# vlc-robot/robot-3dlotus

Hardware: AMD Instinct MI355X
Metric: keystep-samples/sec (train fwd+bwd) 3D-LOTUS GemBench (higher is better)
Workload: dtype f32; 1 GPU; 3D-LOTUS v1 (68.18M params), 16 key-step clouds x 4096 pts per GPU, fwd+loss+bwd, train mode (dropout on), fp32 exact (MFMA f32); global_batch=16, parallelism=dp1, rccl_ranks=0

## Files before the change

robot-3dlotus_amd/csrc/attention.hip:

```cpp
#include "mma.h"
#include <stdlib.h>

namespace LOTUS_NS {

#define AT 128
#define ALD 33
#define SLD 129

struct AttnP {
  const act_t* q; long q_ld; int q_off;
  const act_t* kv; long kv_ld; int k_off, v_off;
  const int* qidx;
  const int* kidx;
  const int* owner;
  const int* tiles;
  const int* blocks;
  const float* qn_w; const float* qn_b; const float* kn_w; const float* kn_b;
  act_t* out; long out_ld;
  float* lse;
  const act_t* dout;
  act_t* dq; long dq_ld; int dq_off;
  act_t* dkv; long dkv_ld; int dk_off, dv_off; long dkv_part_stride;
  float* ln_part;
  int atomic_out;
  const int* kext;
  act_t* dkv_extra;
  long dkv_extra_ld;
  int H, d;
  float scale, eps;
  unsigned long long drop_seed;
  unsigned drop_thresh;
  float drop_inv_keep;
};

__device__ __forceinline__ bool keep_lo(unsigned lo, unsigned s0, unsigned c2, unsigned thresh) {
  unsigned x = lo * 0x9E3779B1u + s0;
  x ^= c2;
  x ^= x >> 16; x *= 0x7FEB352Du; x ^= x >> 15;
  return x >= thresh;
}

__device__ __forceinline__ f32x16 zero16() {
  f32x16 z;
#pragma unroll
  for (int r = 0; r < 16; ++r) z[r] = 0.f;
  return z;
}

// ... 47 lines not shown
  }
  float* x = img + row * ALD;
  float m = 0.f;
  for (int j = 0; j < d; ++j) m += x[j];
  m /= d;
  float v = 0.f;
  for (int j = 0; j < d; ++j) {
    const float c = x[j] - m;
    v += c * c;
  }
  const float rs = rsqrtf(v / d + eps);
  rstd_s[row] = rs;
  for (int j = 0; j < d; ++j) {
    const float xh = (x[j] - m) * rs;
    x[j] = AFFINE ? xh * g_s[j] + b_s[j] : xh;
  }
}

struct AttnSmem {
  float* Q; float* K; float* V; float* dO; float* S;
  float* qrstd; float* krstd; float* Dv; float* lse;
  float* gq; float* bq; float* gk; float* bk;
  int* qrow; int* krow; int* qown; int* kext;
};

__device__ __forceinline__ AttnSmem carve(float* base, bool bwd) {
  AttnSmem s;
  float* p = base;
  s.Q = p; p += AT * ALD;
  s.K = p; p += AT * ALD;
// ... 43 lines not shown
    else
      l[q] = 0u;
  }
  hi = make_uint4(h[0], h[1], h[2], h[3]);
  lo = make_uint4(l[0], l[1], l[2], l[3]);
}
template <int PREC>
__device__ __forceinline__ f32x16 mfma_split(const uint4& ah, const uint4& al, const uint4& bh, const uint4& bl, f32x16 acc) {
  if (PREC == 3) {
    acc = __builtin_amdgcn_mfma_f32_32x32x16_bf16(__builtin_bit_cast(abf16x8, al), __builtin_bit_cast(abf16x8, bh), acc, 0, 0, 0);
    acc = __builtin_amdgcn_mfma_f32_32x32x16_bf16(__builtin_bit_cast(abf16x8, ah), __builtin_bit_cast(abf16x8, bl), acc, 0, 0, 0);
  }
  return __builtin_amdgcn_mfma_f32_32x32x16_bf16(__builtin_bit_cast(abf16x8, ah), __builtin_bit_cast(abf16x8, bh), acc, 0, 0, 0);
}

template <int PREC, bool NORM = true>
__global__ __launch_bounds__(256, 3) void attn_fwd_kernel(AttnP p) {
  static_assert(NORM || PREC == 0, "the no-norm variant exists in exact fp32 only");
  extern __shared__ __attribute__((aligned(16))) float smem[];
  AttnSmem s = carve(smem, false);
  const int tid = threadIdx.x, wave = tid >> 6, l31 = tid & 31, hh = (tid >> 5) & 1;
  const int h = blockIdx.y, d = p.d;
  const int q_start = p.tiles[blockIdx.x * 4 + 0], q_len = p.tiles[blockIdx.x * 4 + 1];
  const int k_start = p.tiles[blockIdx.x * 4 + 2], k_len = p.tiles[blockIdx.x * 4 + 3];

  if (tid < AT) {
    s.qrow[tid] = tid < q_len ? (p.qidx ? p.qidx[q_start + tid] : q_start + tid) : -1;
    s.krow[tid] = tid < k_len ? (p.kidx ? p.kidx[k_start + tid] : k_start + tid) : -1;
    s.qown[tid] = tid < q_len ? (p.owner ? p.owner[q_start + tid] : 1) : 0;
  }
  if constexpr (NORM) load_affine(p, s);
  __syncthreads();
  {
    const RowSrc src[3] = {{s.Q, p.q, p.q_ld, p.q_off + h * d, s.qrow, q_len}, {s.K, p.kv, p.kv_ld, p.k_off + h * d, s.krow, k_len},
                           {s.V, p.kv, p.kv_ld, p.v_off + h * d, s.krow, k_len}};
    load_rows_batch<3>(src, d);
  }
  __syncthreads();
  if constexpr (NORM) {
    if (tid < AT) ln_rows<true>(s.Q, s.qrstd, tid, q_len, d, p.eps, s.gq, s.bq);
    else ln_rows<true>(s.K, s.krstd, tid - AT, k_len, d, p.eps, s.gk, s.bk);
    __syncthreads();
  }

  const int r0 = wave * 32;
  if (r0 >= q_len) return;
  const int ktiles = (k_len + 31) / 32;
  const int qi = r0 + l31;
  f32x16 acc[4];
#pragma unroll
  for (int t = 0; t < 4; ++t) acc[t] = zero16();
  if constexpr (PREC != 0) {
    uint4 qh[2], ql[2];
#pragma unroll
    for (int q2 = 0; q2 < 2; ++q2) {
      float v[8];
#pragma unroll
      for (int e = 0; e < 8; ++e) v[e] = s.Q[qi * ALD + q2 * 16 + hh * 8 + e];
// ... 31 lines not shown
      acc[t][r] = v;
      m = fmaxf(m, v);
    }
  m = fmaxf(m, __shfl_xor(m, 32, 64));
  float sum = 0.f;
#pragma unroll
  for (int t = 0; t < 4; ++t)
#pragma unroll
    for (int r = 0; r < 16; ++r) {
      const float e = acc[t][r] > -INFINITY ? __expf(acc[t][r] - m) : 0.f;
      acc[t][r] = e;
      sum += e;
    }
  sum += __shfl_xor(sum, 32, 64);
  const float inv = sum > 0.f ? 1.f / sum : 0.f;
  if (p.drop_thresh) {
    const unsigned long long rb = (((unsigned long long)blockIdx.x * p.H + h) * AT + qi) * AT;
    const unsigned lo0 = (unsigned)rb, c2 = (unsigned)(rb >> 32) * 0x7FEB352Du + (unsigned)(p.drop_seed >> 32);
    const unsigned s0 = (unsigned)p.drop_seed;
    const float keep = inv * p.drop_inv_keep;
#pragma unroll
    for (int t = 0; t < 4; ++t)
#pragma unroll
      for (int r = 0; r < 16; ++r)
        acc[t][r] *= keep_lo(lo0 + (unsigned)(t * 32 + (r & 3) + 8 * (r >> 2) + 4 * hh), s0, c2, p.drop_thresh) ? keep : 0.f;
  } else {
#pragma unroll
    for (int t = 0; t < 4; ++t)
#pragma unroll
      for (int r = 0; r < 16; ++r) acc[t][r] *= inv;
// ... 21 lines not shown
#pragma unroll
        for (int r = 0; r < 16; ++r) {
          const int key = t * 32 + (r & 3) + 8 * (r >> 2) + 4 * hh;
          o = __builtin_amdgcn_mfma_f32_32x32x2f32(s.V[key * ALD + l31], acc[t][r], o, 0, 0, 0);
        }
      }
    }
  if (qi < q_len && s.qown[qi]) {
    act_t* orow = p.out + (long)s.qrow[qi] * p.out_ld + h * d;
#pragma unroll
    for (int q4 = 0; q4 < 4; ++q4) {
      const int dc = 8 * q4 + 4 * hh;
      if (dc < d) st4(orow + dc, make_float4(o[4 * q4], o[4 * q4 + 1], o[4 * q4 + 2], o[4 * q4 + 3]));
    }
  }
}

__device__ __forceinline__ void store_rows(const float* img, act_t* base, long ld, int coff, const int* rows_s,
                                           const int* own_s, int len, int d, int atomic, const int* ext_s = nullptr,
                                           act_t* ext_base = nullptr, long ext_ld = 0, int ext_coff = 0) {
  const int sub = threadIdx.x & 7;
  for (int r = threadIdx.x >> 3; r < len; r += 32) {
    if (own_s && !own_s[r]) continue;
    if (sub * 4 >= d) continue;
    const float* v = img + r * ALD + sub * 4;
    act_t* o = base + (long)rows_s[r] * ld + coff + sub * 4;
    if (ext_s && ext_s[r] >= 0) o = ext_base + (long)ext_s[r] * ext_ld + ext_coff + sub * 4;
#if !LOTUS_ACT_IS_BF16
    if (atomic) {
#pragma unroll
// ... 8 lines not shown
__device__ __forceinline__ void ln_rows_bwd(float* g, const float* xh, const float* rstd_s, int row, int len, int d,
                                            const float* gam) {
  if (row >= len) return;
  float* gr = g + row * ALD;
  const float* xr = xh + row * ALD;
  float s1 = 0.f, s2 = 0.f;
  for (int j = 0; j < d; ++j) {
    const float t = gr[j] * gam[j];
    s1 += t;
    s2 += t * xr[j];
  }
  s1 /= d;
  s2 /= d;
  const float rs = rstd_s[row];
  for (int j = 0; j < d; ++j) gr[j] = rs * (gr[j] * gam[j] - s1 - xr[j] * s2);
}

template <int PREC>
__global__ __launch_bounds__(256, 2) void attn_bwd_kernel(AttnP p) {
  extern __shared__ __attribute__((aligned(16))) float smem[];
  AttnSmem s = carve(smem, true);
  __shared__ float lnacc[4][32];
  __shared__ float colred[2][8][32];
  const int tid = threadIdx.x, wave = tid >> 6, l31 = tid & 31, hh = (tid >> 5) & 1;
  const int h = blockIdx.y, d = p.d;
  const int* bd = p.blocks + blockIdx.x * 6;
  const int first_tile = bd[0], n_tiles = bd[1], tile_step = bd[2], part_slot = bd[3];
  const int k_start = bd[4], k_len = bd[5];
  const int r0 = wave * 32;
  const int ktiles = (k_len + 31) / 32;
// ... 352 lines not shown
  }
  if (tid < AT) ln_rows_bwd(s.dO, s.K, s.krstd, tid, k_len, d, s.gk);
  __syncthreads();
  act_t* dkv = p.dkv + (long)part_slot * p.dkv_part_stride;
  store_rows(s.dO, dkv, p.dkv_ld, p.dk_off + h * d, s.krow, nullptr, k_len, d, p.atomic_out, p.dkv_extra ? s.kext : nullptr,
             p.dkv_extra, p.dkv_extra_ld, h * d);
  store_rows(s.V, dkv, p.dkv_ld, p.dv_off + h * d, s.krow, nullptr, k_len, d, p.atomic_out, p.dkv_extra ? s.kext : nullptr,
             p.dkv_extra, p.dkv_extra_ld, p.dv_off - p.dk_off + h * d);
  if (tid < 128) p.ln_part[((long)(blockIdx.x * p.H + h) * 4 + (tid >> 5)) * 32 + (tid & 31)] = lnacc[tid >> 5][tid & 31];
}

typedef float f32x4v __attribute__((ext_vector_type(4)));

__device__ __forceinline__ int xswz(int key) { return ((key & 1) << 2) | ((key >> 1) & 3); }

template <bool NORM = true>
__global__ __launch_bounds__(256, 2) void attn_bwd2_kernel(AttnP p) {
  extern __shared__ __attribute__((aligned(16))) float smem[];
  AttnSmem s = carve(smem, true);
  __shared__ float lnacc[NORM ? 4 : 1][32];
  __shared__ float colred[NORM ? 2 : 1][NORM ? 8 : 1][32];
  const int tid = threadIdx.x, wave = tid >> 6, lane = tid & 63, l31 = tid & 31, hh = (tid >> 5) & 1;
  const int h = blockIdx.y, d = p.d;
  const int* bd = p.blocks + blockIdx.x * 6;
  const int first_tile = bd[0], n_tiles = bd[1], tile_step = bd[2], part_slot = bd[3];
  const int k_start = bd[4], k_len = bd[5];
  const int r0 = wave * 32;
  const int ktiles = (k_len + 31) / 32;
  float* X = s.V;

  if (tid < AT) {
    s.krow[tid] = tid < k_len ? (p.kidx ? p.kidx[k_start + tid] : k_start + tid) : -1;
    s.kext[tid] = (tid < k_len && p.kext) ? p.kext[k_start + tid] : -1;
  }
  if constexpr (NORM) {
    if (tid < 4 * 32) lnacc[tid >> 5][tid & 31] = 0.f;
    load_affine(p, s);
  }
  __syncthreads();
  {
    const RowSrc src[2] = {{s.K, p.kv, p.kv_ld, p.k_off + h * d, s.krow, k_len}, {s.V, p.kv, p.kv_ld, p.v_off + h * d, s.krow, k_len}};
    load_rows_batch<2>(src, d);
  }
  __syncthreads();
  if constexpr (NORM) {
    if (tid >= AT) ln_rows<false>(s.K, s.krstd, tid - AT, k_len, d, p.eps, nullptr, nullptr);
    __syncthreads();
  }

  const float gq_l = NORM ? s.gq[l31] : 1.f, bq_l = NORM ? s.bq[l31] : 0.f;
  const float sl2 = p.scale * 1.4426950408889634f;
  const bool has_keys = r0 < k_len;
  const int kj = r0 + l31;
  float kb[16], vb[16], c_a = 0.f;
  if (has_keys) {
#pragma unroll
    for (int s2 = 0; s2 < 16; ++s2) {
      const int k = 2 * s2 + hh;
      if constexpr (NORM) {
        const float kn = s.K[kj * ALD + k] * s.gk[k] + s.bk[k];
        c_a += s.bq[k] * kn;
        kb[s2] = kn * s.gq[k] * sl2;
      } else {
        kb[s2] = s.K[kj * ALD + k] * sl2;
      }
      vb[s2] = s.V[kj * ALD + k];
    }
    if constexpr (NORM) {
      c_a += __shfl_xor(c_a, 32, 64);
      c_a = kj < k_len ? c_a * sl2 : -INFINITY;
    } else {
      c_a = kj < k_len ? 0.f : -INFINITY;
    }
  }
  f32x16 acc_dv = zero16(), acc_dk = zero16();
  const int dh = wave & 1, qh = wave >> 1, l15 = lane & 15, kq = lane >> 4;
  const float gk_c = NORM ? s.gk[16 * dh + l15] : 1.f, bk_c = NORM ? s.bk[16 * dh + l15] : 0.f;
  __syncthreads();

  for (int ti = 0; ti < n_tiles; ++ti) {
    const int tile = first_tile + ti * tile_step;
    const int q_start = p.tiles[tile * 4 + 0], q_len = p.tiles[tile * 4 + 1];
    if (tid < AT) {
      s.qrow[tid] = tid < q_len ? (p.qidx ? p.qidx[q_start + tid] : q_start + tid) : -1;
      s.qown[tid] = tid < q_len ? (p.owner ? p.owner[q_start + tid] : 1) : 0;
      s.lse[tid] = tid < q_len ? p.lse[(long)(q_start + tid) * p.H + h] * 1.4426950408889634f : INFINITY;
    }
    __syncthreads();
    {
      const int sub = tid & 7, rr0 = tid >> 3;
      float4 qv[4], gv[4], ov[4];
#pragma unroll
      for (int j = 0; j < 4; ++j) {
        const int r = rr0 + 32 * j;
        qv[j] = gv[j] = ov[j] = make_float4(0.f, 0.f, 0.f, 0.f);
        if (r < q_len && sub * 4 < d) {
          qv[j] = ld4(p.q + (long)s.qrow[r] * p.q_ld + p.q_off + h * d + sub * 4);
          if (s.qown[r]) {
            const long o = (long)s.qrow[r] * p.out_ld + h * d + sub * 4;
            gv[j] = ld4(p.dout + o);
            ov[j] = ld4(p.out + o);
          }
        }
      }
#pragma unroll
      for (int j = 0; j < 4; ++j) {
        const int r = rr0 + 32 * j;
        float* oq = s.Q + r * ALD + sub * 4;
        oq[0] = qv[j].x; oq[1] = qv[j].y; oq[2] = qv[j].z; oq[3] = qv[j].w;
        float* o = s.dO + r * ALD + sub * 4;
        o[0] = gv[j].x; o[1] = gv[j].y; o[2] = gv[j].z; o[3] = gv[j].w;
        float dsum = gv[j].x * ov[j].x + gv[j].y * ov[j].y + gv[j].z * ov[j].z + gv[j].w * ov[j].w;
        dsum += __shfl_xor(dsum, 1, 64);
        dsum += __shfl_xor(dsum, 2, 64);
        dsum += __shfl_xor(dsum, 4, 64);
        if (sub == 0) s.Dv[r] = dsum;
      }
    }
    __syncthreads();
    if constexpr (NORM) {
      if (tid < AT) ln_rows<false>(s.Q, s.qrstd, tid, q_len, d, p.eps, nullptr, nullptr);
      __syncthreads();
    }

    const unsigned long long tb = ((unsigned long long)tile * p.H + h) * AT * AT;
    const unsigned c2 = (unsigned)(tb >> 32) * 0x7FEB352Du + (unsigned)(p.drop_seed >> 32);
    const unsigned x_lane = ((unsigned)tb + (unsigned)kj + (unsigned)(4 * hh * AT)) * 0x9E3779B1u + (unsigned)p.drop_seed;
    const int qtiles = (q_len + 31) / 32;
    for (int qt = 0; qt < qtiles; ++qt) {
      f32x16 sa, dpa;
      if (has_keys) {
#pragma unroll
        for (int r = 0; r < 16; ++r) { sa[r] = c_a; dpa[r] = 0.f; }
        const float* qrow_p = s.Q + (qt * 32 + l31) * ALD + hh;
        const float* dorow_p = s.dO + (qt * 32 + l31) * ALD + hh;
#pragma unroll
        for (int s2 = 0; s2 < 16; ++s2) {
          sa = __builtin_amdgcn_mfma_f32_32x32x2f32(qrow_p[2 * s2], kb[s2], sa, 0, 0, 0);
// ... 50 lines not shown
        const float* kcol = s.K + 16 * dh + l15;
        for (int t = 0; t < ktiles; ++t) {
#pragma unroll
          for (int s4 = 0; s4 < 8; ++s4) {
            const int key = 32 * t + 4 * s4 + kq;
            const float a = NORM ? kcol[key * ALD] * gk_c + bk_c : kcol[key * ALD];
            const float b = X[key * 32 + ((((ql >> 2) ^ xswz(key)) << 2) | (ql & 3))];
            acc = __builtin_amdgcn_mfma_f32_16x16x4f32(a, b, acc, 0, 0, 0);
          }
        }
        float* o = s.dO + (qt * 32 + ql) * ALD + 16 * dh + 4 * kq;
        o[0] = acc[0]; o[1] = acc[1]; o[2] = acc[2]; o[3] = acc[3];
      }
    }
    __syncthreads();
    if constexpr (NORM) {
      const int j = tid & 31, part = tid >> 5;
      float ag = 0.f, ab = 0.f;
      if (j < d)
        for (int r = part * 16; r < min(q_len, part * 16 + 16); ++r) {
          const float g = s.dO[r * ALD + j];
          ag += g * s.Q[r * ALD + j];
          ab += g;
        }
      colred[0][part][j] = ag;
      colred[1][part][j] = ab;
    }
    if constexpr (NORM) {
      __syncthreads();
      if (tid < 64) {
        const int which = tid >> 5, j = tid & 31;
        float a = 0.f;
        for (int k = 0; k < 8; ++k) a += colred[which][k][j];
        lnacc[which][j] += a;
      }
      if (tid < AT) ln_rows_bwd(s.dO, s.Q, s.qrstd, tid, q_len, d, s.gq);
      __syncthreads();
    }
    store_rows(s.dO, p.dq, p.dq_ld, p.dq_off + h * d, s.qrow, s.qown, q_len, d, 0);
    __syncthreads();
  }

#pragma unroll
  for (int r = 0; r < 16; ++r) {
    const int dc = (r & 3) + 8 * (r >> 2) + 4 * hh;
    s.V[(r0 + l31) * ALD + dc] = (dc < d) ? acc_dv[r] : 0.f;
    s.dO[(r0 + l31) * ALD + dc] = (dc < d) ? acc_dk[r] : 0.f;
  }
  __syncthreads();
  if constexpr (NORM) {
    const int j = tid & 31, part = tid >> 5;
    float ag = 0.f, ab = 0.f;
    if (j < d)
      for (int r = part * 16; r < min(k_len, part * 16 + 16); ++r) {
        const float g = s.dO[r * ALD + j];
        ag += g * s.K[r * ALD + j];
        ab += g;
      }
    colred[0][part][j] = ag;
    colred[1][part][j] = ab;
  }
  if constexpr (NORM) {
    __syncthreads();
    if (tid < 64) {
      const int which = tid >> 5, j = tid & 31;
      float a = 0.f;
      for (int k = 0; k < 8; ++k) a += colred[which][k][j];
      lnacc[2 + which][j] = a;
    }
    if (tid < AT) ln_rows_bwd(s.dO, s.K, s.krstd, tid, k_len, d, s.gk);
    __syncthreads();
  }
  act_t* dkv = p.dkv + (long)part_slot * p.dkv_part_stride;
  store_rows(s.dO, dkv, p.dkv_ld, p.dk_off + h * d, s.krow, nullptr, k_len, d, p.atomic_out, p.dkv_extra ? s.kext : nullptr,
             p.dkv_extra, p.dkv_extra_ld, h * d);
  store_rows(s.V, dkv, p.dkv_ld, p.dv_off + h * d, s.krow, nullptr, k_len, d, p.atomic_out, p.dkv_extra ? s.kext : nullptr,
             p.dkv_extra, p.dkv_extra_ld, p.dv_off - p.dk_off + h * d);
  if constexpr (NORM)
    if (tid < 128) p.ln_part[((long)(blockIdx.x * p.H + h) * 4 + (tid >> 5)) * 32 + (tid & 31)] = lnacc[tid >> 5][tid & 31];
}

__global__ __launch_bounds__(1024) void attn_ln_reduce_kernel(const float* __restrict__ part, float* o0, float* o1,
                                                              float* o2, float* o3, int nb, int d, int accumulate) {
  __shared__ float red[32][33];
  const int which = blockIdx.x, j = threadIdx.x & 31, r = threadIdx.x >> 5;
  float s = 0.f;
  int b = r;
  for (; b + 96 < nb; b += 128) {
    const float v0 = part[((long)b * 4 + which) * 32 + j], v1 = part[((long)(b + 32) * 4 + which) * 32 + j];
    const float v2 = part[((long)(b + 64) * 4 + which) * 32 + j], v3 = part[((long)(b + 96) * 4 + which) * 32 + j];
    s += (v0 + v1) + (v2 + v3);
  }
  for (; b < nb; b += 32) s += part[((long)b * 4 + which) * 32 + j];
  red[r][j] = s;
// ... 770 lines not shown
  for (int g = 0; g < 4; ++g)
    st4(op + 8 * g, make_float4(aO[4 * g] * inv, aO[4 * g + 1] * inv, aO[4 * g + 2] * inv, aO[4 * g + 3] * inv));
}

static int xq_mode() {
  static int on = -1;
  if (on < 0) { const char* e = getenv("LOTUS_XQ"); on = e ? atoi(e) : 1; }
  return on;
}
static bool xq_ok(int k_max, int precision, int atomic_out, int d) {
  const bool geom = !atomic_out && (d == 32 || d == 24 || d == 16);
  const bool short_keys = k_max > 0 && k_max <= 32;
  return geom && ((short_keys && xq_mode() >= 1) || (!short_keys && precision == 0 && !LOTUS_ACT_IS_BF16 && xq_mode() == 2));
}

static int check_geom(int H, int d) { return (d % 4 == 0 && d <= 32 && d >= 4 && H > 0) ? 0 : -1; }

static int norm_mode(const float* qn_w, const float* qn_b, const float* kn_w, const float* kn_b) {
  const int n = (qn_w != nullptr) + (qn_b != nullptr) + (kn_w != nullptr) + (kn_b != nullptr);
  return n == 4 ? 1 : n == 0 ? 0 : -1;
}
#define LOTUS_CHECK_NO_NORM(name, precision)                                                                                \
  do {                                                                                                                     \
    LOTUS_CHECK_ARG(!LOTUS_ACT_IS_BF16, name ": attention without q/k norm (null qn_w, qn_b, kn_w, kn_b) is not built for " \
                                             "bf16 activation storage");                                                   \
    LOTUS_CHECK_ARG((precision) == 0, name ": attention without q/k norm (null qn_w, qn_b, kn_w, kn_b) is built for "       \
                                           "precision 0 (fp32) only, got precision %d", (int)(precision));                 \
  } while (0)

extern "C" {

int lotus_attention_fwd(const act_t* q, long q_ld, int q_off, const act_t* kv, long kv_ld, int k_off, int v_off,
                        const int* qidx, const int* kidx, const int* owner, const int* tiles, int ntiles,
                        const float* qn_w, const float* qn_b, const float* kn_w, const float* kn_b, act_t* out,
                        long out_ld, float* lse, int H, int d, float scale, float eps, float drop_p,
                        unsigned long long drop_seed, int precision, int k_max, void* stream) {
  LOTUS_CHECK_ARG(q && kv && tiles && out && check_geom(H, d) == 0, "lotus_attention_fwd: bad arguments (H=%d d=%d)", H, d);
  const int norm = norm_mode(qn_w, qn_b, kn_w, kn_b);
  LOTUS_CHECK_ARG(norm >= 0, "lotus_attention_fwd: bad arguments (qn_w, qn_b, kn_w, kn_b must be all given or all null)");
  if (!norm) LOTUS_CHECK_NO_NORM("lotus_attention_fwd", precision);
  if (ntiles == 0) return LOTUS_OK;
  AttnP p;
  memset(&p, 0, sizeof(p));
  p.q = q; p.q_ld = q_ld; p.q_off = q_off; p.kv = kv; p.kv_ld = kv_ld; p.k_off = k_off; p.v_off = v_off;
  p.qidx = qidx; p.kidx = kidx; p.owner = owner; p.tiles = tiles;
  p.qn_w = qn_w; p.qn_b = qn_b; p.kn_w = kn_w; p.kn_b = kn_b;
  p.out = out; p.out_ld = out_ld; p.lse = lse; p.H = H; p.d = d; p.scale = scale; p.eps = eps;
  set_attn_drop(p, drop_p, drop_seed);
  if (!norm) {
    const size_t sm = attn_smem_bytes(false);
    const auto attn_fwd_plain = attn_fwd_kernel<0, false>;
    { static bool a0 = false; if (!a0) { (void)hipFuncSetAttribute((const void*)attn_fwd_plain, hipFuncAttributeMaxDynamicSharedMemorySize, (int)sm); a0 = true; } }
    LOTUS_LAUNCH(attn_fwd_plain, dim3(ntiles, H), dim3(256), sm, (hipStream_t)stream, p);
    LOTUS_LAUNCH_CHECK("lotus_attention_fwd(no q/k norm)");
    return LOTUS_OK;
  }
  if (xq_ok(k_max, precision, 0, d)) {
    if (d == 32 && k_max > 0 && k_max <= 32 && !owner && xq_mode() != 3)
      LOTUS_LAUNCH(xq2_fwd_kernel<4>, dim3(ntiles, H), dim3(256), 0, (hipStream_t)stream, p);
    else if (d == 32) LOTUS_LAUNCH(xq_fwd_kernel<32>, dim3(ntiles, H), dim3(128), 0, (hipStream_t)stream, p);
    else if (d == 24) LOTUS_LAUNCH(xq_fwd_kernel<24>, dim3(ntiles, H), dim3(128), 0, (hipStream_t)stream, p);
    else LOTUS_LAUNCH(xq_fwd_kernel<16>, dim3(ntiles, H), dim3(128), 0, (hipStream_t)stream, p);
    LOTUS_LAUNCH_CHECK("lotus_attention_fwd(query per lane)");
    return LOTUS_OK;
  }
  const size_t sm = attn_smem_bytes(false);
  const int prec = precision;
  if (prec == 3) {
    { static bool a1 = false; if (!a1) { (void)hipFuncSetAttribute((const void*)attn_fwd_kernel<3>, hipFuncAttributeMaxDynamicSharedMemorySize, (int)sm); a1 = true; } }
    LOTUS_LAUNCH(attn_fwd_kernel<3>, dim3(ntiles, H), dim3(256), sm, (hipStream_t)stream, p);
  } else if (prec == 1) {
    { static bool a2 = false; if (!a2) { (void)hipFuncSetAttribute((const void*)attn_fwd_kernel<1>, hipFuncAttributeMaxDynamicSharedMemorySize, (int)sm); a2 = true; } }
    LOTUS_LAUNCH(attn_fwd_kernel<1>, dim3(ntiles, H), dim3(256), sm, (hipStream_t)stream, p);
  } else {
    { static bool a3 = false; if (!a3) { (void)hipFuncSetAttribute((const void*)attn_fwd_kernel<0>, hipFuncAttributeMaxDynamicSharedMemorySize, (int)sm); a3 = true; } }
    LOTUS_LAUNCH(attn_fwd_kernel<0>, dim3(ntiles, H), dim3(256), sm, (hipStream_t)stream, p);
  }
  LOTUS_LAUNCH_CHECK("lotus_attention_fwd");
  return LOTUS_OK;
}

size_t lotus_attention_bwd_workspace(int nblocks, int H) { return (size_t)nblocks * H * 4 * 32 * sizeof(float); }

int lotus_attention_bwd(const act_t* q, long q_ld, int q_off, const act_t* kv, long kv_ld, int k_off, int v_off,
                        const int* qidx, const int* kidx, const int* owner, const int* tiles, const int* blocks,
                        int nblocks, const float* qn_w, const float* qn_b, const float* kn_w, const float* kn_b,
                        const act_t* out, const act_t* dout, long out_ld, const float* lse, act_t* dq, long dq_ld,
                        int dq_off, act_t* dkv, long dkv_ld, int dk_off, int dv_off, long dkv_part_stride,
                        int atomic_out, const int* kext, const int* ext_pos, int n_extra, act_t* dkv_extra, float* dqn_w, float* dqn_b, float* dkn_w, float* dkn_b, int accumulate,
                        int H, int d, float scale, float eps, float drop_p, unsigned long long drop_seed,
                        int precision, int k_max, void* workspace, size_t workspace_bytes, void* stream) {
// ... 8 lines not shown
  if (nblocks == 0) return LOTUS_OK;
  AttnP p;
  memset(&p, 0, sizeof(p));
  p.q = q; p.q_ld = q_ld; p.q_off = q_off; p.kv = kv; p.kv_ld = kv_ld; p.k_off = k_off; p.v_off = v_off;
  p.qidx = qidx; p.kidx = kidx; p.owner = owner; p.tiles = tiles; p.blocks = blocks;
  p.qn_w = qn_w; p.qn_b = qn_b; p.kn_w = kn_w; p.kn_b = kn_b;
  p.out = (act_t*)out; p.dout = dout; p.out_ld = out_ld; p.lse = (float*)lse;
  p.dq = dq; p.dq_ld = dq_ld; p.dq_off = dq_off;
  p.dkv = dkv; p.dkv_ld = dkv_ld; p.dk_off = dk_off; p.dv_off = dv_off; p.dkv_part_stride = dkv_part_stride;
  p.atomic_out = atomic_out; p.ln_part = (float*)workspace;
  p.kext = kext; p.dkv_extra = (kext && n_extra > 0) ? dkv_extra : nullptr; p.dkv_extra_ld = 2L * H * d;
  LOTUS_CHECK_ARG(!(kext && n_extra > 0) || (dkv_extra && ext_pos && dv_off - dk_off == H * d),
                  "lotus_attention_bwd: borrowed-row buffer needs dkv_extra, ext_pos and adjacent k|v column blocks");
  p.H = H; p.d = d; p.scale = scale; p.eps = eps;
  set_attn_drop(p, drop_p, drop_seed);
  hipStream_t st = (hipStream_t)stream;
  const size_t sm = attn_smem_bytes(true);
  const int prec = precision;
  StopEventOnLast stop_ev;
  if (!norm) {
    { static bool a7 = false; if (!a7) { (void)hipFuncSetAttribute((const void*)attn_bwd2_kernel<false>, hipFuncAttributeMaxDynamicSharedMemorySize, (int)sm); a7 = true; } }
    if (!p.dkv_extra) stop_ev.last();
    LOTUS_LAUNCH(attn_bwd2_kernel<false>, dim3(nblocks, H), dim3(256), sm, st, p);
    if (p.dkv_extra) {
      const int w4 = 2 * H * d / 4;
      stop_ev.last();
      LOTUS_LAUNCH(attn_extra_fixup_kernel, dim3(cdiv((long)n_extra * w4, 256)), dim3(256), 0, st, dkv_extra, 2L * H * d,
                         ext_pos, kidx, n_extra, w4, dkv, dkv_ld, dk_off);
    }
    LOTUS_LAUNCH_CHECK("lotus_attention_bwd(no q/k norm)");
    return LOTUS_OK;
  }
  if (xq_ok(k_max, precision, atomic_out, d)) {
    if (d == 32 && k_max > 0 && k_max <= 32 && !owner && !p.dkv_extra && xq_mode() != 3)
      LOTUS_LAUNCH(xq2_bwd_kernel<4>, dim3(nblocks, H), dim3(256), 0, st, p);
    else if (d == 32) LOTUS_LAUNCH(xq_bwd_kernel<32>, dim3(nblocks, H), dim3(128), 0, st, p);
    else if (d == 24) LOTUS_LAUNCH(xq_bwd_kernel<24>, dim3(nblocks, H), dim3(128), 0, st, p);
    else LOTUS_LAUNCH(xq_bwd_kernel<16>, dim3(nblocks, H), dim3(128), 0, st, p);
  } else if (prec == 3) {
    { static bool a4 = false; if (!a4) { (void)hipFuncSetAttribute((const void*)attn_bwd_kernel<3>, hipFuncAttributeMaxDynamicSharedMemorySize, (int)sm); a4 = true; } }
    LOTUS_LAUNCH(attn_bwd_kernel<3>, dim3(nblocks, H), dim3(256), sm, st, p);
  } else if (prec == 1) {
    { static bool a5 = false; if (!a5) { (void)hipFuncSetAttribute((const void*)attn_bwd_kernel<1>, hipFuncAttributeMaxDynamicSharedMemorySize, (int)sm); a5 = true; } }
    LOTUS_LAUNCH(attn_bwd_kernel<1>, dim3(nblocks, H), dim3(256), sm, st, p);
  } else {
    { static bool a6 = false; if (!a6) { (void)hipFuncSetAttribute((const void*)attn_bwd2_kernel<true>, hipFuncAttributeMaxDynamicSharedMemorySize, (int)sm); a6 = true; } }
    LOTUS_LAUNCH(attn_bwd2_kernel<true>, dim3(nblocks, H), dim3(256), sm, st, p);
  }
  if (p.dkv_extra) {
    const int w4 = 2 * H * d / 4;
    LOTUS_LAUNCH(attn_extra_fixup_kernel, dim3(cdiv((long)n_extra * w4, 256)), dim3(256), 0, st, dkv_extra, 2L * H * d,
                       ext_pos, kidx, n_extra, w4, dkv, dkv_ld, dk_off);
  }
  stop_ev.last();
  LOTUS_LAUNCH(attn_ln_reduce_kernel, dim3(4), dim3(1024), 0, st, p.ln_part, dqn_w, dqn_b, dkn_w, dkn_b,
                     nblocks * H, d, accumulate);
  LOTUS_LAUNCH_CHECK("lotus_attention_bwd");
  return LOTUS_OK;
}

}

// ... 2 lines not shown
```

Measured before the change: 1082 keystep-samples/s.

## Add single-tile fast path to attention backward and specialize head width at compile time

Adds a one-tile path to the fp32 attention backward kernel: when a key block has exactly one query tile, K/V/Q/dO loads and the D=dO·O reduction happen together, and the barriers and separate per-tile reload are skipped. The K-side layer-norm backward is then overlapped with the dq store and dk/dv written directly. Forward and backward fp32 kernels also get compile-time head widths (16/24/32) so the per-element loops can be fully unrolled. Layer-norm helpers are rewritten with fixed fma contraction, and optional clock64 timestamp probes are added behind a compile flag. Costs are more template instances, extra shared memory for a second column-reduction buffer, and a more complex control flow.

```diff
diff --git a/robot-3dlotus_amd/csrc/attention.hip b/robot-3dlotus_amd/csrc/attention.hip
--- a/robot-3dlotus_amd/csrc/attention.hip
+++ b/robot-3dlotus_amd/csrc/attention.hip
@@ -6,6 +6,12 @@
 #define AT 128
 #define ALD 33
 #define SLD 129
+
+#if defined(LOTUS_ATTN_STAMPS) && !LOTUS_ACT_IS_BF16
+#define ATTN_STAMPS_ON 1
+#else
+#define ATTN_STAMPS_ON 0
+#endif
 
 struct AttnP {
   const act_t* q; long q_ld; int q_off;
@@ -31,7 +37,20 @@
   unsigned long long drop_seed;
   unsigned drop_thresh;
   float drop_inv_keep;
+  int one_tile;
+#if ATTN_STAMPS_ON
+  long long* stamps;
+#endif
 };
+
+#if ATTN_STAMPS_ON
+#define ATTN_STAMP(i)                                                                                                     \
+  do {                                                                                                                    \
+    if (p.stamps && threadIdx.x == 0) p.stamps[((long)blockIdx.y * gridDim.x + blockIdx.x) * 16 + (i)] = clock64();       \
+  } while (0)
+#else
+#define ATTN_STAMP(i) do {} while (0)
+#endif
 
 __device__ __forceinline__ bool keep_lo(unsigned lo, unsigned s0, unsigned c2, unsigned thresh) {
   unsigned x = lo * 0x9E3779B1u + s0;
@@ -109,6 +128,31 @@
   for (int j = 0; j < d; ++j) {
     const float xh = (x[j] - m) * rs;
     x[j] = AFFINE ? xh * g_s[j] + b_s[j] : xh;
+  }
+}
+
+template <bool AFFINE>
+__device__ __forceinline__ void ln_rows_fixed(float* img, float* rstd_s, int row, int len, int d, float eps,
+                                              const float* g_s, const float* b_s) {
+#pragma clang fp contract(off)
+  if (row >= len) {
+    if (row < AT) rstd_s[row] = 0.f;
+    return;
+  }
+  float* x = img + row * ALD;
+  float m = 0.f;
+  for (int j = 0; j < d; ++j) m += x[j];
+  m /= d;
+  float v = 0.f;
+  for (int j = 0; j < d; ++j) {
+    const float c = x[j] - m;
+    v = __builtin_fmaf(c, c, v);
+  }
+  const float rs = rsqrtf(v / d + eps);
+  rstd_s[row] = rs;
+  for (int j = 0; j < d; ++j) {
+    const float xh = (x[j] - m) * rs;
+    x[j] = AFFINE ? __builtin_fmaf(xh, g_s[j], b_s[j]) : xh;
   }
 }
 
@@ -182,13 +226,15 @@
   return __builtin_amdgcn_mfma_f32_32x32x16_bf16(__builtin_bit_cast(abf16x8, ah), __builtin_bit_cast(abf16x8, bh), acc, 0, 0, 0);
 }
 
-template <int PREC, bool NORM = true>
+template <int PREC, bool NORM = true, int DW = 0>
 __global__ __launch_bounds__(256, 3) void attn_fwd_kernel(AttnP p) {
   static_assert(NORM || PREC == 0, "the no-norm variant exists in exact fp32 only");
+  static_assert(DW == 0 || PREC == 0, "the compile-time head width exists in exact fp32 only");
   extern __shared__ __attribute__((aligned(16))) float smem[];
   AttnSmem s = carve(smem, false);
   const int tid = threadIdx.x, wave = tid >> 6, l31 = tid & 31, hh = (tid >> 5) & 1;
-  const int h = blockIdx.y, d = p.d;
+  const int h = blockIdx.y, d = DW ? DW : p.d;
+  ATTN_STAMP(0);
   const int q_start = p.tiles[blockIdx.x * 4 + 0], q_len = p.tiles[blockIdx.x * 4 + 1];
   const int k_start = p.tiles[blockIdx.x * 4 + 2], k_len = p.tiles[blockIdx.x * 4 + 3];
 
@@ -199,17 +245,25 @@
   }
   if constexpr (NORM) load_affine(p, s);
   __syncthreads();
+  ATTN_STAMP(1);
   {
     const RowSrc src[3] = {{s.Q, p.q, p.q_ld, p.q_off + h * d, s.qrow, q_len}, {s.K, p.kv, p.kv_ld, p.k_off + h * d, s.krow, k_len},
                            {s.V, p.kv, p.kv_ld, p.v_off + h * d, s.krow, k_len}};
     load_rows_batch<3>(src, d);
   }
   __syncthreads();
+  ATTN_STAMP(2);
   if constexpr (NORM) {
-    if (tid < AT) ln_rows<true>(s.Q, s.qrstd, tid, q_len, d, p.eps, s.gq, s.bq);
-    else ln_rows<true>(s.K, s.krstd, tid - AT, k_len, d, p.eps, s.gk, s.bk);
-    __syncthreads();
-  }
+    if constexpr (PREC == 0) {
+      if (tid < AT) ln_rows_fixed<true>(s.Q, s.qrstd, tid, q_len, d, p.eps, s.gq, s.bq);
+      else ln_rows_fixed<true>(s.K, s.krstd, tid - AT, k_len, d, p.eps, s.gk, s.bk);
+    } else {
+      if (tid < AT) ln_rows<true>(s.Q, s.qrstd, tid, q_len, d, p.eps, s.gq, s.bq);
+      else ln_rows<true>(s.K, s.krstd, tid - AT, k_len, d, p.eps, s.gk, s.bk);
+    }
+    __syncthreads();
+  }
+  ATTN_STAMP(3);
 
   const int r0 = wave * 32;
   if (r0 >= q_len) return;
@@ -271,6 +325,7 @@
     }
   sum += __shfl_xor(sum, 32, 64);
   const float inv = sum > 0.f ? 1.f / sum : 0.f;
+  ATTN_STAMP(4);
   if (p.drop_thresh) {
     const unsigned long long rb = (((unsigned long long)blockIdx.x * p.H + h) * AT + qi) * AT;
     const unsigned lo0 = (unsigned)rb, c2 = (unsigned)(rb >> 32) * 0x7FEB352Du + (unsigned)(p.drop_seed >> 32);
@@ -322,6 +377,7 @@
       if (dc < d) st4(orow + dc, make_float4(o[4 * q4], o[4 * q4 + 1], o[4 * q4 + 2], o[4 * q4 + 3]));
     }
   }
+  ATTN_STAMP(5);
 }
 
 __device__ __forceinline__ void store_rows(const float* img, act_t* base, long ld, int coff, const int* rows_s,
@@ -360,6 +416,43 @@
   s2 /= d;
   const float rs = rstd_s[row];
   for (int j = 0; j < d; ++j) gr[j] = rs * (gr[j] * gam[j] - s1 - xr[j] * s2);
+}
+
+__device__ __forceinline__ void ln_rows_bwd_fixed(float* g, const float* xh, const float* rstd_s, int row, int len, int d,
+                                                  const float* gam) {
+#pragma clang fp contract(off)
+  if (row >= len) return;
+  float* gr = g + row * ALD;
+  const float* xr = xh + row * ALD;
+  float s1 = 0.f, s2 = 0.f;
+  for (int j = 0; j < d; ++j) {
+    const float t = gr[j] * gam[j];
+    s1 += t;
+    s2 += t * xr[j];
+  }
+  s1 /= d;
+  s2 /= d;
+  const float rs = rstd_s[row];
+  for (int j = 0; j < d; ++j) gr[j] = rs * __builtin_fmaf(-s2, xr[j], __builtin_fmaf(gr[j], gam[j], -s1));
+}
+
+__device__ __forceinline__ void col_partials(const float* g, const float* xh, int len, int d, float (*red)[8][32]) {
+#pragma clang fp contract(off)
+  const int j = threadIdx.x & 31, part = threadIdx.x >> 5;
+  float ag = 0.f, ab = 0.f;
+  if (j < d)
+    for (int r = part * 16; r < min(len, part * 16 + 16); ++r) {
+      const float v = g[r * ALD + j];
+      ag += v * xh[r * ALD + j];
+      ab += v;
+    }
+  red[0][part][j] = ag;
+  red[1][part][j] = ab;
+}
+
+__device__ __forceinline__ float dot4(const float4& a, const float4& b) {
+#pragma clang fp contract(off)
+  return a.x * b.x + a.y * b.y + a.z * b.z + a.w * b.w;
 }
 
 template <int PREC>
@@ -742,39 +835,99 @@
 
 __device__ __forceinline__ int xswz(int key) { return ((key & 1) << 2) | ((key >> 1) & 3); }
 
-template <bool NORM = true>
+template <bool NORM = true, int DW = 0>
 __global__ __launch_bounds__(256, 2) void attn_bwd2_kernel(AttnP p) {
   extern __shared__ __attribute__((aligned(16))) float smem[];
   AttnSmem s = carve(smem, true);
   __shared__ float lnacc[NORM ? 4 : 1][32];
   __shared__ float colred[NORM ? 2 : 1][NORM ? 8 : 1][32];
+  __shared__ float colred_k[NORM ? 2 : 1][NORM ? 8 : 1][32];
   const int tid = threadIdx.x, wave = tid >> 6, lane = tid & 63, l31 = tid & 31, hh = (tid >> 5) & 1;
-  const int h = blockIdx.y, d = p.d;
+  const int h = blockIdx.y, d = DW ? DW : p.d;
+  ATTN_STAMP(0);
   const int* bd = p.blocks + blockIdx.x * 6;
   const int first_tile = bd[0], n_tiles = bd[1], tile_step = bd[2], part_slot = bd[3];
   const int k_start = bd[4], k_len = bd[5];
   const int r0 = wave * 32;
   const int ktiles = (k_len + 31) / 32;
   float* X = s.V;
+  const bool one = n_tiles == 1 && p.one_tile;
 
   if (tid < AT) {
     s.krow[tid] = tid < k_len ? (p.kidx ? p.kidx[k_start + tid] : k_start + tid) : -1;
     s.kext[tid] = (tid < k_len && p.kext) ? p.kext[k_start + tid] : -1;
+    if (one) {
+      const int q_start = p.tiles[first_tile * 4 + 0], q_len = p.tiles[first_tile * 4 + 1];
+      s.qrow[tid] = tid < q_len ? (p.qidx ? p.qidx[q_start + tid] : q_start + tid) : -1;
+      s.qown[tid] = tid < q_len ? (p.owner ? p.owner[q_start + tid] : 1) : 0;
+      s.lse[tid] = tid < q_len ? p.lse[(long)(q_start + tid) * p.H + h] * 1.4426950408889634f : INFINITY;
+    }
   }
   if constexpr (NORM) {
     if (tid < 4 * 32) lnacc[tid >> 5][tid & 31] = 0.f;
     load_affine(p, s);
   }
   __syncthreads();
-  {
-    const RowSrc src[2] = {{s.K, p.kv, p.kv_ld, p.k_off + h * d, s.krow, k_len}, {s.V, p.kv, p.kv_ld, p.v_off + h * d, s.krow, k_len}};
-    load_rows_batch<2>(src, d);
-  }
-  __syncthreads();
-  if constexpr (NORM) {
-    if (tid >= AT) ln_rows<false>(s.K, s.krstd, tid - AT, k_len, d, p.eps, nullptr, nullptr);
-    __syncthreads();
-  }
+  ATTN_STAMP(1);
+  if (one) {
+    const int q_len = p.tiles[first_tile * 4 + 1];
+    const int sub = tid & 7, rr0 = tid >> 3;
+    float4 kv[4], vv[4], qv[4], gv[4], ov[4];
+#pragma unroll
+    for (int j = 0; j < 4; ++j) {
+      const int r = rr0 + 32 * j;
+      kv[j] = vv[j] = qv[j] = gv[j] = ov[j] = make_float4(0.f, 0.f, 0.f, 0.f);
+      if (r < k_len && sub * 4 < d) {
+        const act_t* row = p.kv + (long)s.krow[r] * p.kv_ld + h * d + sub * 4;
+        kv[j] = ld4(row + p.k_off);
+        vv[j] = ld4(row + p.v_off);
+      }
+      if (r < q_len && sub * 4 < d) {
+        qv[j] = ld4(p.q + (long)s.qrow[r] * p.q_ld + p.q_off + h * d + sub * 4);
+        if (s.qown[r]) {
+          const long o = (long)s.qrow[r] * p.out_ld + h * d + sub * 4;
+          gv[j] = ld4(p.dout + o);
+          ov[j] = ld4(p.out + o);
+        }
+      }
+    }
+#pragma unroll
+    for (int j = 0; j < 4; ++j) {
+      const int r = rr0 + 32 * j;
+      float* o = s.K + r * ALD + sub * 4;
+      o[0] = kv[j].x; o[1] = kv[j].y; o[2] = kv[j].z; o[3] = kv[j].w;
+      o = s.V + r * ALD + sub * 4;
+      o[0] = vv[j].x; o[1] = vv[j].y; o[2] = vv[j].z; o[3] = vv[j].w;
+      o = s.Q + r * ALD + sub * 4;
+      o[0] = qv[j].x; o[1] = qv[j].y; o[2] = qv[j].z; o[3] = qv[j].w;
+      o = s.dO + r * ALD + sub * 4;
+      o[0] = gv[j].x; o[1] = gv[j].y; o[2] = gv[j].z; o[3] = gv[j].w;
+      float dsum = dot4(gv[j], ov[j]);
+      dsum += __shfl_xor(dsum, 1, 64);
+      dsum += __shfl_xor(dsum, 2, 64);
+      dsum += __shfl_xor(dsum, 4, 64);
+      if (sub == 0) s.Dv[r] = dsum;
+    }
+    __syncthreads();
+    ATTN_STAMP(2);
+    if constexpr (NORM) {
+      if (tid < AT) ln_rows_fixed<false>(s.Q, s.qrstd, tid, q_len, d, p.eps, nullptr, nullptr);
+      else ln_rows_fixed<false>(s.K, s.krstd, tid - AT, k_len, d, p.eps, nullptr, nullptr);
+      __syncthreads();
+    }
+  } else {
+    {
+      const RowSrc src[2] = {{s.K, p.kv, p.kv_ld, p.k_off + h * d, s.krow, k_len}, {s.V, p.kv, p.kv_ld, p.v_off + h * d, s.krow, k_len}};
+      load_rows_batch<2>(src, d);
+    }
+    __syncthreads();
+    ATTN_STAMP(2);
+    if constexpr (NORM) {
+      if (tid >= AT) ln_rows_fixed<false>(s.K, s.krstd, tid - AT, k_len, d, p.eps, nullptr, nullptr);
+      __syncthreads();
+    }
+  }
+  ATTN_STAMP(3);
 
   const float gq_l = NORM ? s.gq[l31] : 1.f, bq_l = NORM ? s.bq[l31] : 0.f;
   const float sl2 = p.scale * 1.4426950408889634f;
@@ -804,52 +957,56 @@
   f32x16 acc_dv = zero16(), acc_dk = zero16();
   const int dh = wave & 1, qh = wave >> 1, l15 = lane & 15, kq = lane >> 4;
   const float gk_c = NORM ? s.gk[16 * dh + l15] : 1.f, bk_c = NORM ? s.bk[16 * dh + l15] : 0.f;
-  __syncthreads();
+  if (!one) __syncthreads();
+  ATTN_STAMP(4);
 
   for (int ti = 0; ti < n_tiles; ++ti) {
     const int tile = first_tile + ti * tile_step;
     const int q_start = p.tiles[tile * 4 + 0], q_len = p.tiles[tile * 4 + 1];
-    if (tid < AT) {
-      s.qrow[tid] = tid < q_len ? (p.qidx ? p.qidx[q_start + tid] : q_start + tid) : -1;
-      s.qown[tid] = tid < q_len ? (p.owner ? p.owner[q_start + tid] : 1) : 0;
-      s.lse[tid] = tid < q_len ? p.lse[(long)(q_start + tid) * p.H + h] * 1.4426950408889634f : INFINITY;
-    }
-    __syncthreads();
-    {
-      const int sub = tid & 7, rr0 = tid >> 3;
-      float4 qv[4], gv[4], ov[4];
-#pragma unroll
-      for (int j = 0; j < 4; ++j) {
-        const int r = rr0 + 32 * j;
-        qv[j] = gv[j] = ov[j] = make_float4(0.f, 0.f, 0.f, 0.f);
-        if (r < q_len && sub * 4 < d) {
-          qv[j] = ld4(p.q + (long)s.qrow[r] * p.q_ld + p.q_off + h * d + sub * 4);
-          if (s.qown[r]) {
-            const long o = (long)s.qrow[r] * p.out_ld + h * d + sub * 4;
-            gv[j] = ld4(p.dout + o);
-            ov[j] = ld4(p.out + o);
-          }
-        }
-      }
-#pragma unroll
-      for (int j = 0; j < 4; ++j) {
-        const int r = rr0 + 32 * j;
-        float* oq = s.Q + r * ALD + sub * 4;
-        oq[0] = qv[j].x; oq[1] = qv[j].y; oq[2] = qv[j].z; oq[3] = qv[j].w;
-        float* o = s.dO + r * ALD + sub * 4;
-        o[0] = gv[j].x; o[1] = gv[j].y; o[2] = gv[j].z; o[3] = gv[j].w;
-        float dsum = gv[j].x * ov[j].x + gv[j].y * ov[j].y + gv[j].z * ov[j].z + gv[j].w * ov[j].w;
-        dsum += __shfl_xor(dsum, 1, 64);
-        dsum += __shfl_xor(dsum, 2, 64);
-        dsum += __shfl_xor(dsum, 4, 64);
-        if (sub == 0) s.Dv[r] = dsum;
-      }
-    }
-    __syncthreads();
-    if constexpr (NORM) {
-      if (tid < AT) ln_rows<false>(s.Q, s.qrstd, tid, q_len, d, p.eps, nullptr, nullptr);
+    if (!one) {
+      if (tid < AT) {
+        s.qrow[tid] = tid < q_len ? (p.qidx ? p.qidx[q_start + tid] : q_start + tid) : -1;
+        s.qown[tid] = tid < q_len ? (p.owner ? p.owner[q_start + tid] : 1) : 0;
+        s.lse[tid] = tid < q_len ? p.lse[(long)(q_start + tid) * p.H + h] * 1.4426950408889634f : INFINITY;
+      }
       __syncthreads();
-    }
+      {
+        const int sub = tid & 7, rr0 = tid >> 3;
+        float4 qv[4], gv[4], ov[4];
+#pragma unroll
+        for (int j = 0; j < 4; ++j) {
+          const int r = rr0 + 32 * j;
+          qv[j] = gv[j] = ov[j] = make_float4(0.f, 0.f, 0.f, 0.f);
+          if (r < q_len && sub * 4 < d) {
+            qv[j] = ld4(p.q + (long)s.qrow[r] * p.q_ld + p.q_off + h * d + sub * 4);
+            if (s.qown[r]) {
+              const long o = (long)s.qrow[r] * p.out_ld + h * d + sub * 4;
+              gv[j] = ld4(p.dout + o);
+              ov[j] = ld4(p.out + o);
+            }
+          }
+        }
+#pragma unroll
+        for (int j = 0; j < 4; ++j) {
+          const int r = rr0 + 32 * j;
+          float* oq = s.Q + r * ALD + sub * 4;
+          oq[0] = qv[j].x; oq[1] = qv[j].y; oq[2] = qv[j].z; oq[3] = qv[j].w;
+          float* o = s.dO + r * ALD + sub * 4;
+          o[0] = gv[j].x; o[1] = gv[j].y; o[2] = gv[j].z; o[3] = gv[j].w;
+          float dsum = dot4(gv[j], ov[j]);
+          dsum += __shfl_xor(dsum, 1, 64);
+          dsum += __shfl_xor(dsum, 2, 64);
+          dsum += __shfl_xor(dsum, 4, 64);
+          if (sub == 0) s.Dv[r] = dsum;
+        }
+      }
+      __syncthreads();
+      if constexpr (NORM) {
+        if (tid < AT) ln_rows_fixed<false>(s.Q, s.qrstd, tid, q_len, d, p.eps, nullptr, nullptr);
+        __syncthreads();
+      }
+    }
+    ATTN_STAMP(5);
 
     const unsigned long long tb = ((unsigned long long)tile * p.H + h) * AT * AT;
     const unsigned c2 = (unsigned)(tb >> 32) * 0x7FEB352Du + (unsigned)(p.drop_seed >> 32);
@@ -930,19 +1087,10 @@
       }
     }
     __syncthreads();
+    ATTN_STAMP(6);
+    if (one) break;
     if constexpr (NORM) {
-      const int j = tid & 31, part = tid >> 5;
-      float ag = 0.f, ab = 0.f;
-      if (j < d)
-        for (int r = part * 16; r < min(q_len, part * 16 + 16); ++r) {
-          const float g = s.dO[r * ALD + j];
-          ag += g * s.Q[r * ALD + j];
-          ab += g;
-        }
-      colred[0][part][j] = ag;
-      colred[1][part][j] = ab;
-    }
-    if constexpr (NORM) {
+      col_partials(s.dO, s.Q, q_len, d, colred);
       __syncthreads();
       if (tid < 64) {
         const int which = tid >> 5, j = tid & 31;
@@ -950,11 +1098,65 @@
         for (int k = 0; k < 8; ++k) a += colred[which][k][j];
         lnacc[which][j] += a;
       }
-      if (tid < AT) ln_rows_bwd(s.dO, s.Q, s.qrstd, tid, q_len, d, s.gq);
+      if (tid < AT) ln_rows_bwd_fixed(s.dO, s.Q, s.qrstd, tid, q_len, d, s.gq);
       __syncthreads();
     }
     store_rows(s.dO, p.dq, p.dq_ld, p.dq_off + h * d, s.qrow, s.qown, q_len, d, 0);
     __syncthreads();
+    ATTN_STAMP(7);
+  }
+
+  if (one) {
+    const int q_len = p.tiles[first_tile * 4 + 1];
+    float* G = s.V;
+    act_t* dkv = p.dkv + (long)part_slot * p.dkv_part_stride;
+#pragma unroll
+    for (int r = 0; r < 16; ++r) {
+      const int dc = (r & 3) + 8 * (r >> 2) + 4 * hh;
+      G[(r0 + l31) * ALD + dc] = (dc < d) ? acc_dk[r] : 0.f;
+    }
+    if (kj < k_len) {
+      act_t* o = dkv + (long)s.krow[kj] * p.dkv_ld + p.dv_off + h * d;
+      if (p.dkv_extra && s.kext[kj] >= 0) o = p.dkv_extra + (long)s.kext[kj] * p.dkv_extra_ld + p.dv_off - p.dk_off + h * d;
+#pragma unroll
+      for (int q4 = 0; q4 < 4; ++q4) {
+        const int dc = 8 * q4 + 4 * hh;
+        if (dc < d) st4(o + dc, make_float4(acc_dv[4 * q4], acc_dv[4 * q4 + 1], acc_dv[4 * q4 + 2], acc_dv[4 * q4 + 3]));
+      }
+    }
+    if constexpr (NORM) {
+      col_partials(s.dO, s.Q, q_len, d, colred);
+      __syncthreads();
+      col_partials(G, s.K, k_len, d, colred_k);
+      if (tid < AT) {
+        ln_rows_bwd_fixed(s.dO, s.Q, s.qrstd, tid, q_len, d, s.gq);
+      } else if (tid < AT + 64) {
+        const int which = (tid - AT) >> 5, j = tid & 31;
+        float a = 0.f;
+        for (int k = 0; k < 8; ++k) a += colred[which][k][j];
+        lnacc[which][j] += a;
+      }
+    }
+    __syncthreads();
+    ATTN_STAMP(7);
+    store_rows(s.dO, p.dq, p.dq_ld, p.dq_off + h * d, s.qrow, s.qown, q_len, d, 0);
+    if constexpr (NORM) {
+      if (tid >= AT) {
+        ln_rows_bwd_fixed(G, s.K, s.krstd, tid - AT, k_len, d, s.gk);
+      } else if (tid < 64) {
+        const int which = tid >> 5, j = tid & 31;
+        float a = 0.f;
+        for (int k = 0; k < 8; ++k) a += colred_k[which][k][j];
+        lnacc[2 + which][j] = a;
+      }
+      __syncthreads();
+    }
+    store_rows(G, dkv, p.dkv_ld, p.dk_off + h * d, s.krow, nullptr, k_len, d, 0, p.dkv_extra ? s.kext : nullptr, p.dkv_extra,
+               p.dkv_extra_ld, h * d);
+    if constexpr (NORM)
+      if (tid < 128) p.ln_part[((long)(blockIdx.x * p.H + h) * 4 + (tid >> 5)) * 32 + (tid & 31)] = lnacc[tid >> 5][tid & 31];
+    ATTN_STAMP(8);
+    return;
   }
 
 #pragma unroll
@@ -965,18 +1167,7 @@
   }
   __syncthreads();
   if constexpr (NORM) {
-    const int j = tid & 31, part = tid >> 5;
-    float ag = 0.f, ab = 0.f;
-    if (j < d)
-      for (int r = part * 16; r < min(k_len, part * 16 + 16); ++r) {
-        const float g = s.dO[r * ALD + j];
-        ag += g * s.K[r * ALD + j];
-        ab += g;
-      }
-    colred[0][part][j] = ag;
-    colred[1][part][j] = ab;
-  }
-  if constexpr (NORM) {
+    col_partials(s.dO, s.K, k_len, d, colred);
     __syncthreads();
     if (tid < 64) {
       const int which = tid >> 5, j = tid & 31;
@@ -984,7 +1175,7 @@
       for (int k = 0; k < 8; ++k) a += colred[which][k][j];
       lnacc[2 + which][j] = a;
     }
-    if (tid < AT) ln_rows_bwd(s.dO, s.K, s.krstd, tid, k_len, d, s.gk);
+    if (tid < AT) ln_rows_bwd_fixed(s.dO, s.K, s.krstd, tid, k_len, d, s.gk);
     __syncthreads();
   }
   act_t* dkv = p.dkv + (long)part_slot * p.dkv_part_stride;
@@ -994,6 +1185,7 @@
              p.dkv_extra, p.dkv_extra_ld, p.dv_off - p.dk_off + h * d);
   if constexpr (NORM)
     if (tid < 128) p.ln_part[((long)(blockIdx.x * p.H + h) * 4 + (tid >> 5)) * 32 + (tid & 31)] = lnacc[tid >> 5][tid & 31];
+  ATTN_STAMP(8);
 }
 
 __global__ __launch_bounds__(1024) void attn_ln_reduce_kernel(const float* __restrict__ part, float* o0, float* o1,
@@ -1794,6 +1986,39 @@
   return geom && ((short_keys && xq_mode() >= 1) || (!short_keys && precision == 0 && !LOTUS_ACT_IS_BF16 && xq_mode() == 2));
 }
 
+static int one_tile_mode() {
+  static int on = -1;
+  if (on < 0) { const char* e = getenv("LOTUS_ATTN_ONE_TILE"); on = e ? (atoi(e) != 0) : 1; }
+  return on;
+}
+
+#if ATTN_STAMPS_ON
+static long long* g_attn_stamps = nullptr;
+#endif
+
+template <void (*KERN)(AttnP)>
+static void launch_tile(dim3 grid, size_t sm, hipStream_t st, const AttnP& p) {
+  static bool raised = false;
+  if (!raised) { (void)hipFuncSetAttribute((const void*)KERN, hipFuncAttributeMaxDynamicSharedMemorySize, (int)sm); raised = true; }
+  LOTUS_LAUNCH(KERN, grid, dim3(256), sm, st, p);
+}
+template <bool NORM>
+static void launch_fwd_fp32(dim3 grid, hipStream_t st, const AttnP& p) {
+  const size_t sm = attn_smem_bytes(false);
+  if (p.d == 32) launch_tile<attn_fwd_kernel<0, NORM, 32>>(grid, sm, st, p);
+  else if (p.d == 24) launch_tile<attn_fwd_kernel<0, NORM, 24>>(grid, sm, st, p);
+  else if (p.d == 16) launch_tile<attn_fwd_kernel<0, NORM, 16>>(grid, sm, st, p);
+  else launch_tile<attn_fwd_kernel<0, NORM, 0>>(grid, sm, st, p);
+}
+template <bool NORM>
+static void launch_bwd2(dim3 grid, hipStream_t st, const AttnP& p) {
+  const size_t sm = attn_smem_bytes(true);
+  if (p.d == 32) launch_tile<attn_bwd2_kernel<NORM, 32>>(grid, sm, st, p);
+  else if (p.d == 24) launch_tile<attn_bwd2_kernel<NORM, 24>>(grid, sm, st, p);
+  else if (p.d == 16) launch_tile<attn_bwd2_kernel<NORM, 16>>(grid, sm, st, p);
+  else launch_tile<attn_bwd2_kernel<NORM, 0>>(grid, sm, st, p);
+}
+
 static int check_geom(int H, int d) { return (d % 4 == 0 && d <= 32 && d >= 4 && H > 0) ? 0 : -1; }
 
 static int norm_mode(const float* qn_w, const float* qn_b, const float* kn_w, const float* kn_b) {
@@ -1809,6 +2034,10 @@
   } while (0)
 
 extern "C" {
+
+#if ATTN_STAMPS_ON
+void lotus_attention_lab_stamps(void* buf) { g_attn_stamps = (long long*)buf; }
+#endif
 
 int lotus_attention_fwd(const act_t* q, long q_ld, int q_off, const act_t* kv, long kv_ld, int k_off, int v_off,
                         const int* qidx, const int* kidx, const int* owner, const int* tiles, int ntiles,
@@ -1827,11 +2056,11 @@
   p.qn_w = qn_w; p.qn_b = qn_b; p.kn_w = kn_w; p.kn_b = kn_b;
   p.out = out; p.out_ld = out_ld; p.lse = lse; p.H = H; p.d = d; p.scale = scale; p.eps = eps;
   set_attn_drop(p, drop_p, drop_seed);
+#if ATTN_STAMPS_ON
+  p.stamps = g_attn_stamps;
+#endif
   if (!norm) {
-    const size_t sm = attn_smem_bytes(false);
-    const auto attn_fwd_plain = attn_fwd_kernel<0, false>;
-    { static bool a0 = false; if (!a0) { (void)hipFuncSetAttribute((const void*)attn_fwd_plain, hipFuncAttributeMaxDynamicSharedMemorySize, (int)sm); a0 = true; } }
-    LOTUS_LAUNCH(attn_fwd_plain, dim3(ntiles, H), dim3(256), sm, (hipStream_t)stream, p);
+    launch_fwd_fp32<false>(dim3(ntiles, H), (hipStream_t)stream, p);
     LOTUS_LAUNCH_CHECK("lotus_attention_fwd(no q/k norm)");
     return LOTUS_OK;
   }
@@ -1853,8 +2082,7 @@
     { static bool a2 = false; if (!a2) { (void)hipFuncSetAttribute((const void*)attn_fwd_kernel<1>, hipFuncAttributeMaxDynamicSharedMemorySize, (int)sm); a2 = true; } }
     LOTUS_LAUNCH(attn_fwd_kernel<1>, dim3(ntiles, H), dim3(256), sm, (hipStream_t)stream, p);
   } else {
-    { static bool a3 = false; if (!a3) { (void)hipFuncSetAttribute((const void*)attn_fwd_kernel<0>, hipFuncAttributeMaxDynamicSharedMemorySize, (int)sm); a3 = true; } }
-    LOTUS_LAUNCH(attn_fwd_kernel<0>, dim3(ntiles, H), dim3(256), sm, (hipStream_t)stream, p);
+    launch_fwd_fp32<true>(dim3(ntiles, H), (hipStream_t)stream, p);
   }
   LOTUS_LAUNCH_CHECK("lotus_attention_fwd");
   return LOTUS_OK;
@@ -1893,14 +2121,17 @@
                   "lotus_attention_bwd: borrowed-row buffer needs dkv_extra, ext_pos and adjacent k|v column blocks");
   p.H = H; p.d = d; p.scale = scale; p.eps = eps;
   set_attn_drop(p, drop_p, drop_seed);
+  p.one_tile = one_tile_mode() && !atomic_out;
+#if ATTN_STAMPS_ON
+  p.stamps = g_attn_stamps;
+#endif
   hipStream_t st = (hipStream_t)stream;
   const size_t sm = attn_smem_bytes(true);
   const int prec = precision;
   StopEventOnLast stop_ev;
   if (!norm) {
-    { static bool a7 = false; if (!a7) { (void)hipFuncSetAttribute((const void*)attn_bwd2_kernel<false>, hipFuncAttributeMaxDynamicSharedMemorySize, (int)sm); a7 = true; } }
     if (!p.dkv_extra) stop_ev.last();
-    LOTUS_LAUNCH(attn_bwd2_kernel<false>, dim3(nblocks, H), dim3(256), sm, st, p);
+    launch_bwd2<false>(dim3(nblocks, H), st, p);
     if (p.dkv_extra) {
       const int w4 = 2 * H * d / 4;
       stop_ev.last();
@@ -1923,8 +2154,7 @@
     { static bool a5 = false; if (!a5) { (void)hipFuncSetAttribute((const void*)attn_bwd_kernel<1>, hipFuncAttributeMaxDynamicSharedMemorySize, (int)sm); a5 = true; } }
     LOTUS_LAUNCH(attn_bwd_kernel<1>, dim3(nblocks, H), dim3(256), sm, st, p);
   } else {
-    { static bool a6 = false; if (!a6) { (void)hipFuncSetAttribute((const void*)attn_bwd2_kernel<true>, hipFuncAttributeMaxDynamicSharedMemorySize, (int)sm); a6 = true; } }
-    LOTUS_LAUNCH(attn_bwd2_kernel<true>, dim3(nblocks, H), dim3(256), sm, st, p);
+    launch_bwd2<true>(dim3(nblocks, H), st, p);
   }
   if (p.dkv_extra) {
     const int w4 = 2 * H * d / 4;
```

Result: no change. 1082 keystep-samples/s (-0.0%).
